# tspooner/rl_markets

Measured on NVIDIA H100. Metric: env steps/sec (batched LOBs), higher is better.
Workload: dtype f64

## Files before the change

rl_markets_b200/csrc/rlm_api.cu:

```cuda
#include <cuda_runtime.h>
#include <math.h>
#include <stdio.h>
#include <string.h>
#include <algorithm>
#include <mutex>
#include <string>
#include <vector>

#include "rlm.h"
#include "rlm_flow_tables.h"
#include "rlm_rndseq.h"
#include "rlm_kernels.h"
#include <limits.h>
#include <stddef.h>
#include <stdlib.h>

static thread_local std::string g_err;
static int fail(int code, const std::string& msg) { g_err = msg; return code; }
int rlm_set_error_(int code, const std::string& msg) { return fail(code, msg); }
#define CK(expr)                                                                                      \
  do {                                                                                                \
    cudaError_t _e = (expr);                                                                          \
    if (_e != cudaSuccess) return fail((_e == cudaErrorNoDevice || _e == cudaErrorInsufficientDriver) ? RLM_ERR_NO_DEVICE : RLM_ERR_CUDA, \
                                       std::string(#expr) + ": " + cudaGetErrorString(_e));          \
// ... 33 lines not shown
  long long launches = 0;
  double alpha = 0, eps = 0, tau = 1.0;
  int n_sub = 1;
  struct TickGraph { int chunk; DynParams d; cudaGraphExec_t exec; };
  std::vector<TickGraph> graphs;
  bool use_graphs = true, graph_warm = false;
  bool staged = false;
  cudaStream_t sub_stream[RLM_MAX_SUB] = {};
  cudaEvent_t ev_fork = nullptr, ev_join[RLM_MAX_SUB] = {};
  bool rounds = false;
  bool in_rounds = false;
  bool rounds_auto = false;
  int run_seq = 0;
  int round_streams = 1;
  int* h_live = nullptr;
  cudaEvent_t ev_live[RLM_MAX_SUB][2] = {};
  long long rounds_launched = 0, rounds_calls = 0;
};

static const rlm_handle_s* g_params_owner = nullptr;
static std::recursive_mutex g_api_mu;
#define API_LOCK std::lock_guard<std::recursive_mutex> api_lock_(g_api_mu)

static int split_scratch(rlm_handle_s* h, size_t bytes) {
  if (bytes > h->gather_cap) {
    CK(cudaStreamSynchronize(h->stream));
    cudaFree(h->d_gather); if (h->h_gather) cudaFreeHost(h->h_gather);
    h->d_gather = nullptr; h->h_gather = nullptr; h->gather_cap = 0;
    CK(cudaMalloc(&h->d_gather, bytes));
    CK(cudaMallocHost(&h->h_gather, bytes));
// ... 253 lines not shown
  int rc = upload_params(h);
  if (rc != RLM_OK) return rc;
  CK(rlm_launch_init(h->ptr, cfg->n_envs, 0, h->stream));
  CK(rlm_launch_seed(h->ptr, cfg->n_envs, cfg->random_seed, h->stream));
  if (cfg->random_init) CK(rlm_launch_random_init(h->ptr, h->n_policies, h->stream));
  h->alpha = cfg->alpha_start;
  h->eps = (double)cfg->eps_init;
  h->tau = (double)cfg->tau_init;
  memset(&h->dyn, 0, sizeof(h->dyn));
#ifdef RLM_TIMING
  if (const char* s = getenv("RLM_DEBUG_FLAGS")) h->dyn.debug_flags = atoi(s);
#endif
  if (const char* s = getenv("RLM_ENV_HASH")) h->dyn.env_hash = atoi(s) != 0;
  if (const char* s = getenv("RLM_ROUND_CAP")) h->dyn.round_cap = std::max(0, atoi(s));
  CK(cudaDeviceGetAttribute(&h->n_sms, cudaDevAttrMultiProcessorCount, cfg->device));
  CK(cudaMalloc(&h->ptr.ready, (size_t)cfg->n_envs * 4));
  CK(cudaMalloc(&h->ptr.hsum, (size_t)cfg->n_envs * 3 * 32 * 8));
  h->ready_cap = RLM_READY_CAP;
  CK(cudaMalloc(&h->ptr.ready_count, (size_t)2 * RLM_LIVE_OFF * 4));
  CK(cudaMemset(h->ptr.ready_count, 0, (size_t)2 * RLM_LIVE_OFF * 4));
  CK(cudaMalloc(&h->ptr.runctl, sizeof(RunCtl)));
  CK(cudaMemset(h->ptr.runctl, 0, sizeof(RunCtl)));
  CK(cudaMallocHost(&h->h_live, RLM_MAX_SUB * 2 * sizeof(int)));
  for (int s = 0; s < RLM_MAX_SUB; ++s)
    for (int i = 0; i < 2; ++i) CK(cudaEventCreateWithFlags(&h->ev_live[s][i], cudaEventDisableTiming));
  if (const char* s = getenv("RLM_ROUND_STREAMS")) { const int v = atoi(s); if (v >= 1 && v <= RLM_MAX_SUB) h->round_streams = v; }
  h->n_sub = 1;
  h->staged = !h->hp.is_double && !cfg->shared_policy && cfg->memory_size * 8 <= 65536 && (cfg->memory_size % 2) == 0;
  if (const char* s = getenv("RLM_STAGED")) h->staged = h->staged && atoi(s) != 0;
  if (cfg->n_envs > 16384 && !h->staged) h->agent_variant = 3;
  if (const char* s = getenv("RLM_AGENT_VARIANT")) { const int v = atoi(s); h->agent_variant = (v == 1 || v == 3) ? v : 4; }
  if (cfg->memory_size > (1LL << 27) && h->agent_variant == 4) h->agent_variant = 3;
  if (const char* s = getenv("RLM_GRAPHS")) h->use_graphs = atoi(s) != 0;
  if (const char* s = getenv("RLM_SUBBATCHES")) { const int v = atoi(s); if (v >= 1 && v <= RLM_MAX_SUB) h->n_sub = cfg->shared_policy ? 1 : v; }
  if (std::max(h->n_sub, h->round_streams) > 1) {
// ... 21 lines not shown
    const int resident = rlm_run_max_resident_ctas(p.scratch_bytes, h->n_sms);
    const int n_env_ctas = (cfg->n_envs + 127) / 128;
    int want = (cfg->n_envs + 3) / 4;
    int cap = resident - std::min(n_env_ctas, std::max(resident / 4, 1));
    h->n_agent_ctas = std::max(1, std::min(want, cap));
    if (const char* s = getenv("RLM_AGENT_CTAS")) { int v = atoi(s); if (v > 0 && v < resident) h->n_agent_ctas = v; }
    if (const char* s = getenv("RLM_ENGINE")) h->engine = (s[0] == 'p') ? 0 : ((s[0] == 'f') ? 2 : ((s[0] == 'F') ? 3 : 1));
    h->env_variant = (cfg->n_envs > 16384) ? 1 : 0;
    if (const char* s = getenv("RLM_ENV_VARIANT")) h->env_variant = atoi(s) ? 1 : 0;
    h->rounds = false;
    h->rounds_auto = !cfg->shared_policy && h->env_variant == 0 && h->engine == 1 && !getenv("RLM_ENGINE") && cfg->algorithm < RLM_ALGO_R_LEARN;
    if (const char* s = getenv("RLM_ROUNDS")) {
      h->rounds = atoi(s) != 0 && !cfg->shared_policy && h->env_variant == 0;
      h->rounds_auto = false;
    }
    if (!getenv("RLM_ROUND_CAP")) h->dyn.round_cap = 3;
    if (const char* s = getenv("RLM_PDL")) rlm_set_pdl(atoi(s));
    if (const char* s = getenv("RLM_AGENT_VARIANT")) { const int v = atoi(s); h->agent_variant = (v == 1 || v == 3) ? v : 4; }
    if (cfg->memory_size > (1LL << 27)) {
      if (h->agent_variant == 4) h->agent_variant = 3;
      if (h->engine == 3) h->engine = 1;
    }
  }
  if (cfg->source == RLM_SOURCE_TAPE) {
    if (h->engine != 1) return fail(RLM_ERR_UNSUPPORTED, "the tape source runs on the tick-synchronous and round-paced engines (RLM_ENGINE=F|f|p read the stream source only)");
    h->dyn.tape_l2 = 1;
    if (const char* s = getenv("RLM_TAPE_PREFETCH")) h->dyn.tape_l2 = atoi(s) != 0;
  }
  cudaDeviceSetLimit(cudaLimitMaxL2FetchGranularity, 32);
  CK(cudaStreamSynchronize(h->stream));
  return RLM_OK;
}
// ... 2 lines not shown
  API_LOCK;
  if (!h) return RLM_OK;
  cudaSetDevice(h->cfg.device);
  cudaStreamSynchronize(h->stream);
  cudaFree(h->ptr.env); cudaFree(h->ptr.theta); cudaFree(h->ptr.theta_b); cudaFree(h->ptr.dtheta);
  cudaFree(h->ptr.trace_f); cudaFree(h->ptr.trace_e); cudaFree(h->ptr.mt_pol); cudaFree(h->ptr.mt_agt);
  cudaFree(h->ptr.records); cudaFree(h->ptr.record_count); cudaFree(h->ptr.counters);
  cudaFree(h->d_gather); if (h->h_gather) cudaFreeHost(h->h_gather);
  if (h->copy_stream) { cudaStreamSynchronize(h->copy_stream); cudaStreamDestroy(h->copy_stream); }
  for (int i = 0; i < 2; ++i) {
    cudaFree(h->d_stream[i]);
    if (h->ev_copied[i]) cudaEventDestroy(h->ev_copied[i]);
    if (h->ev_consumed[i]) cudaEventDestroy(h->ev_consumed[i]);
  }
  cudaFree(h->ptr.ready); cudaFree(h->ptr.ready_count); cudaFree(h->ptr.occ); cudaFree(h->ptr.hsum);
  cudaFree(h->ptr.runctl); if (h->h_live) cudaFreeHost(h->h_live);
  cudaFree((void*)h->ptr.tape); cudaFree(h->ptr.tape_cur); cudaFree(h->ptr.tape_lo);
  for (auto& es : h->ev_live) for (auto e : es) if (e) cudaEventDestroy(e);
  cudaFree(h->ptr.q_slots); cudaFree(h->ptr.ag_done); cudaFree(h->d_qctl);
  for (auto e : h->ev) cudaEventDestroy(e);
  for (auto& g : h->graphs) cudaGraphExecDestroy(g.exec);
  if (h->ev_fork) cudaEventDestroy(h->ev_fork);
  for (int s = 0; s < RLM_MAX_SUB; ++s) {
    if (h->sub_stream[s]) { cudaStreamSynchronize(h->sub_stream[s]); cudaStreamDestroy(h->sub_stream[s]); }
    if (h->ev_join[s]) cudaEventDestroy(h->ev_join[s]);
  }
  if (h->own_stream && h->stream) cudaStreamDestroy(h->stream);
  if (g_params_owner == h) g_params_owner = nullptr;
  delete h;
  return RLM_OK;
}
// ... 201 lines not shown
  CK(rlm_launch_runctl(h->ptr, rc, h->stream));
  const int S = h->profile ? 1 : std::max(1, std::min(h->round_streams, (B + 255) / 256));
  int sub0[RLM_MAX_SUB + 1];
  {
    const int per = (((B + S - 1) / S) + 31) & ~31;
    for (int s = 0; s <= S; ++s) sub0[s] = std::min(B, s * per);
  }
  int G = n_ticks >= 512 ? 32 : (n_ticks >= 128 ? 16 : 8);
  G = std::min(std::min(G, n_ticks + 1), h->ready_cap);
  const bool graphs = h->use_graphs && h->graph_warm && !h->profile;
  h->graph_warm = true;
  if (h->profile) while ((int)h->ev.size() < 3 * G) { cudaEvent_t e; CK(cudaEventCreate(&e)); h->ev.push_back(e); }
  DynParams dts[RLM_MAX_SUB];
  DevPtrs pss[RLM_MAX_SUB];
  cudaGraphExec_t exec[RLM_MAX_SUB] = {};
  if (S > 1) CK(cudaEventRecord(h->ev_fork, h->stream));
  for (int s = 0; s < S; ++s) {
    cudaStream_t st = S > 1 ? h->sub_stream[s] : h->stream;
    if (S > 1) CK(cudaStreamWaitEvent(st, h->ev_fork, 0));
    DynParams& dt = dts[s];
    dt = d;
    dt.n_ticks = 0; dt.stream_off = 0; dt.stream_ticks = 0; dt.env0 = sub0[s]; dt.n_sub = sub0[s + 1] - sub0[s]; dt.sub_idx = s;
    DevPtrs& ps = pss[s];
    ps = h->ptr;
    ps.stream = nullptr;
    ps.ready = h->ptr.ready + sub0[s];
    ps.ready_count = h->ptr.ready_count + (size_t)s * h->ready_cap;
    if (!graphs || dt.n_sub <= 0) continue;
    for (auto& g : h->graphs)
      if (g.chunk == -G && memcmp(&g.d, &dt, sizeof(DynParams)) == 0) exec[s] = g.exec;
    if (!exec[s]) {
      if (h->graphs.size() >= 24) {
        CK(cudaStreamSynchronize(h->stream));
        for (auto& g : h->graphs) cudaGraphExecDestroy(g.exec);
        h->graphs.clear();
        for (int q = 0; q < s; ++q) exec[q] = nullptr;
      }
      cudaGraph_t graph = nullptr;
      CK(cudaStreamBeginCapture(st, cudaStreamCaptureModeThreadLocal));
      cudaError_t ce = cudaMemsetAsync(ps.ready_count, 0, (size_t)G * 4, st);
      if (ce == cudaSuccess) ce = cudaMemsetAsync(ps.ready_count + RLM_LIVE_OFF, 0, (size_t)G * 4, st);
      for (int r = 0; r < G && ce == cudaSuccess; ++r) {
        ce = rlm_launch_env_round(ps, dt, dt.n_sub, r, st);
        if (ce == cudaSuccess) ce = launch_agent_on(h, ps, dt, r, 0, st);
      }
      cudaError_t ce2 = cudaStreamEndCapture(st, &graph);
      if (ce != cudaSuccess || ce2 != cudaSuccess) { if (graph) cudaGraphDestroy(graph); CK(ce != cudaSuccess ? ce : ce2); }
      ce = cudaGraphInstantiate(&exec[s], graph, 0);
      cudaGraphDestroy(graph);
      CK(ce);
      h->graphs.push_back({-G, dt, exec[s]});
    }
  }
  const int max_groups = (n_ticks + 1 + G - 1) / G + 1;
  bool live[RLM_MAX_SUB];
  int n_live = 0;
  for (int s = 0; s < S; ++s) { live[s] = sub0[s + 1] > sub0[s]; n_live += live[s] ? 1 : 0; }
  h->rounds_calls++;
  for (int k = 0; k <= max_groups && n_live > 0; ++k) {
    for (int s = 0; s < S && k < max_groups; ++s) {
      if (!live[s]) continue;
      cudaStream_t st = S > 1 ? h->sub_stream[s] : h->stream;
      if (exec[s]) CK(cudaGraphLaunch(exec[s], st));
      else {
        CK(cudaMemsetAsync(pss[s].ready_count, 0, (size_t)G * 4, st));
        CK(cudaMemsetAsync(pss[s].ready_count + RLM_LIVE_OFF, 0, (size_t)G * 4, st));
        for (int r = 0; r < G; ++r) {
          if (h->profile) CK(cudaEventRecord(h->ev[3 * r], st));
          CK(rlm_launch_env_round(pss[s], dts[s], dts[s].n_sub, r, st));
          if (h->profile) CK(cudaEventRecord(h->ev[3 * r + 1], st));
          CK(launch_agent_on(h, pss[s], dts[s], r, 0, st));
          if (h->profile) CK(cudaEventRecord(h->ev[3 * r + 2], st));
        }
        if (h->profile) {
          std::vector<int> cnt(2 * G);
          CK(cudaStreamSynchronize(st));
          CK(cudaMemcpy(cnt.data(), pss[s].ready_count, (size_t)G * 4, cudaMemcpyDeviceToHost));
          CK(cudaMemcpy(cnt.data() + G, pss[s].ready_count + RLM_LIVE_OFF, (size_t)G * 4, cudaMemcpyDeviceToHost));
          for (int r = 0; r < G; ++r) {
            float a = 0, b = 0;
            CK(cudaEventElapsedTime(&a, h->ev[3 * r], h->ev[3 * r + 1]));
            CK(cudaEventElapsedTime(&b, h->ev[3 * r + 1], h->ev[3 * r + 2]));
            if (cnt[G + r] > 0) { h->prof_env_ms += a; h->prof_env_launches++; }
            if (cnt[r] > 0) { h->prof_agent_ms += b; h->prof_agent_launches++; }
          }
        }
// ... 654 lines not shown
```

rl_markets_b200/csrc/rlm_kernels.cu:

```cuda
#include <cuda_runtime.h>
#include <stdint.h>
#define RLM_TABLE_QUAL static __device__ const
#include "rlm_flow_tables.h"
#include "rlm_rndseq.h"
#include "rlm_agent.cuh"
#include <cstdio>
#include "rlm_kernels.h"
#define RLM_ENVT_CARVEOUT_DEFAULT 30
#define RLM_SMEM_CARVEOUT 88

#define SCR_Q 0
#define SCR_SS (SCR_Q + 8 * 2 * RLM_MAX_ACTIONS)
#define SCR_IDX (SCR_SS + 4 * SS_SLOTS)
#define SCR_VBUF (SCR_IDX + 4 * 3 * RLM_MAX_ACTIONS * 32)
#define AG_BYTES ((sizeof(AgentD) + 15) & ~(size_t)15)
size_t rlm_scratch_bytes(int is_double) {
  return ((size_t)SCR_VBUF + (size_t)(is_double ? 2 : 1) * RLM_MAX_ACTIONS * VROW * 8 + 15) & ~(size_t)15;
}
size_t rlm_agent_smem_bytes(int warps_per_cta, int scratch_bytes) {
  return (size_t)warps_per_cta * (AG_BYTES + (size_t)scratch_bytes);
}

#define PDL_PROLOGUE() do { asm volatile("griddepcontrol.launch_dependents;" ::: "memory"); asm volatile("griddepcontrol.wait;" ::: "memory"); } while (0)
static bool g_use_pdl = false;
void rlm_set_pdl(int on) { g_use_pdl = on != 0; }
template <typename... KArgs, typename... Args>
static cudaError_t launch_pdl(void (*kernel)(KArgs...), int grid, int block, size_t smem, cudaStream_t st, Args... args) {
  cudaLaunchConfig_t cfg = {};
  cfg.gridDim = dim3(grid); cfg.blockDim = dim3(block); cfg.dynamicSmemBytes = smem; cfg.stream = st;
  cudaLaunchAttribute at[1];
  at[0].id = cudaLaunchAttributeProgrammaticStreamSerialization;
  at[0].val.programmaticStreamSerializationAllowed = g_use_pdl ? 1 : 0;
  cfg.attrs = at; cfg.numAttrs = 1;
  return cudaLaunchKernelEx(&cfg, kernel, args...);
}

#ifdef RLM_TIMING
__device__ unsigned long long g_klog[256][8][2][2];
__device__ __forceinline__ unsigned long long gtime() { unsigned long long t; asm volatile("mov.u64 %0, %%globaltimer;" : "=l"(t)); return t; }
#define KLOG_BEGIN(kind) do { if (threadIdx.x == 0 && tslot < 256) atomicMin(&g_klog[tslot][D.sub_idx & 7][kind][0], gtime()); } while (0)
#define KLOG_END(kind) do { if (threadIdx.x == 0 && tslot < 256) atomicMax(&g_klog[tslot][D.sub_idx & 7][kind][1], gtime()); } while (0)
extern "C" int rlm_debug_klog(unsigned long long* out, int reset) {
  cudaDeviceSynchronize();
  if (out && cudaMemcpyFromSymbol(out, g_klog, sizeof(g_klog)) != cudaSuccess) return -1;
  if (reset) {
    static unsigned long long init[256][8][2][2];
    for (auto& a : init) for (auto& b : a) for (auto& c : b) { c[0] = ~0ull; c[1] = 0ull; }
// ... 730 lines not shown
            }
          }
        }
        if (lane == 0) e.ag.hs_valid = 1;
      }
    } else if (ready == 1 && D.backtest) {
      if (lane < P.n_state_vars) e.ag.to_vars[lane] = (float)get_variable(e, ring, P.state_vars[lane]);
    }
  }
  __syncwarp();
  return ready;
}

template <bool TAPE>
__global__ void __launch_bounds__(ENVW_WARPS * 32) rlm_env_kernel_w(DevPtrs ptr, DynParams D, int tslot, int only_begin) {
  PDL_PROLOGUE();
  extern __shared__ __align__(16) unsigned char smem[];
  const int tid = threadIdx.x, lane = tid & 31, warp = tid >> 5;
  const int env = D.env0 + blockIdx.x * (blockDim.x >> 5) + warp;
  if (!only_begin) KLOG_BEGIN(0);
  if (env >= (D.n_sub > 0 ? D.env0 + D.n_sub : P.n_envs)) return;
  const EnvWarp w = envw_carve(smem + (size_t)warp * envw_warp_bytes());
  EnvHdr& e = *w.e;
  EnvHdr* g = (EnvHdr*)(ptr.env + (size_t)env * P.env_stride);
  double* ring = (double*)((unsigned char*)g + sizeof(EnvHdr));
  if (only_begin && !g->ag.need_begin) return;
  const bool tape = TAPE && !only_begin;
  int2 tc = make_int2(0, 0);
  unsigned tape_word = 0;
  if (tape) tape_word = envw_stage_in_tape(&e, g, ptr, env, lane, D.tape_l2 != 0, tc);
  else envw_stage_in(&e, g, lane);
// ... 22 lines not shown
  }
  __syncwarp();
  envw_stage_out(g, &e, lane);
  if (!only_begin) KLOG_END(0);
  if (lane == 0) {
    if (ready >= 0) ptr.ready[atomicAdd(&ptr.ready_count[tslot], 1)] = env;
    if (D.hold && ready < 0 && e.phase != PH_DONE && !starved) atomicAdd(&ptr.counters[5], 1ull);
    if (ticked) atomicAdd(&ptr.counters[0], 1ull);
    const unsigned errs = (unsigned)(e.err | e.ag.err);
    if (errs) atomicOr(&ptr.counters[4], (unsigned long long)errs);
  }
}

template <bool TAPE>
__global__ void __launch_bounds__(ENVW_WARPS * 32, 4) rlm_env_round_kernel(DevPtrs ptr, DynParams D, int tslot) {
  PDL_PROLOGUE();
  extern __shared__ __align__(16) unsigned char smem[];
  const int tid = threadIdx.x, lane = tid & 31, warp = tid >> 5;
  const int env = D.env0 + blockIdx.x * (blockDim.x >> 5) + warp;
  KLOG_BEGIN(0);
  if (env >= (D.n_sub > 0 ? D.env0 + D.n_sub : P.n_envs)) return;
  int* live_count = ptr.ready_count + RLM_LIVE_OFF;
  if (tslot > 0 && __ldcg(live_count + tslot - 1) == 0) return;
  const int4 rc4 = __ldg((const int4*)ptr.runctl);
  const RunCtl rc = {rc4.x, rc4.y, rc4.z, rc4.w, nullptr, 0};
  DevPtrs pt = ptr;
  pt.stream = (const rlm_tick_msg*)__ldg((const unsigned long long*)ptr.runctl + 2);
  const EnvWarp w = envw_carve(smem + (size_t)warp * envw_warp_bytes());
  EnvHdr& e = *w.e;
  EnvHdr* g = (EnvHdr*)(ptr.env + (size_t)env * P.env_stride);
  double* ring = (double*)((unsigned char*)g + sizeof(EnvHdr));
  const bool tape = TAPE;
  int2 tc = make_int2(0, 0);
  unsigned tape_word = 0;
  if (tape) tape_word = envw_stage_in_tape(&e, g, ptr, env, lane, false, tc);
  else envw_stage_in(&e, g, lane);
  __syncwarp();
  if (e.phase == PH_DONE) return;
// ... 19 lines not shown
    }
    ++pos; ++n_run;
    if (ready >= 0) break;
  }
  if (lane == 0) {
    e.run_id = rc.run_id; e.run_pos = pos;
    if (tape) {
      ptr.tape_cur[env].x = tc.x;
      if (D.tape_l2 && tc.x < tc.y) asm volatile("prefetch.global.L2 [%0];" ::"l"(ptr.tape + tc.x));
    }
  }
  __syncwarp();
  envw_stage_out(g, &e, lane);
  KLOG_END(0);
  if (lane == 0) {
    if (ready >= 0) ptr.ready[atomicAdd(&ptr.ready_count[tslot], 1)] = env;
    if (ready >= 0 || (e.phase != PH_DONE && pos < rc.n_ticks && !starved)) atomicAdd(&live_count[tslot], 1);
    if (ticked) atomicAdd(&ptr.counters[0], (unsigned long long)ticked);
    const unsigned errs = (unsigned)(e.err | e.ag.err);
    if (errs) atomicOr(&ptr.counters[4], (unsigned long long)errs);
  }
}
__global__ void rlm_runctl_kernel(RunCtl* dst, RunCtl v) { *dst = v; }

__device__ __forceinline__ void emit_record(const DevPtrs& ptr, const EnvHdr* g, int env, const AgentD& ag, const double* theta_a,
                                         const float* vars, int lane) {
  const int* tf = ptr.trace_f + (size_t)env * P.trace_cap;
  const float* te = ptr.trace_e + (size_t)env * P.trace_cap;
  unsigned long long h = trace_hash(tf, te, theta_a, ag.n_traces, lane);
  if (lane == 0) {
    int c = ptr.record_count[env];
    if (c < P.record_cap) {
// ... 420 lines not shown
  int f[RLM_MAX_ACTIONS];
  const unsigned long long base = a3_hash(rlm_rndseq_table, ag.to_vars, P.n_state_vars, false, warp, lane, f);
  if (P.occ_smem_words) { asm volatile("cp.async.wait_all;" ::: "memory"); __syncthreads(); }
  a3_gather(theta_a, theta_b, occ, occ_sm, f, warp, lane, V);
  __syncthreads();
  if (warp == 0) {
    double qa = 0.0, qb = 0.0;
    if (lane < P.n_actions) a3_sums(V, theta_b != nullptr, lane, qa, qb);
    backtest_advance(ptr, g, env, ag, theta_a, kind, qa, qb, base, lane, steps_done);
  }
  return (int)steps_done;
}

template <bool EXTRAS>
__global__ void __launch_bounds__(A3_WARPS * 32, 10) rlm_agent3_kernel(DevPtrs ptr, DynParams D, int tslot, int stage) {
  PDL_PROLOGUE();
  extern __shared__ __align__(16) unsigned char smem[];
  const int tid = threadIdx.x, lane = tid & 31, warp = tid >> 5;
  AgentD& ag = *(AgentD*)smem;
  unsigned char* sb = smem + AG_BYTES;
  double* q_pre_a = (double*)(sb + A3_Q);
  double* q_pre_b = q_pre_a + RLM_MAX_ACTIONS;
  int* sset = (int*)(sb + A3_SS);
  double* dec = (double*)(sb + A3_DEC);
  double* V = (double*)(sb + A3_V);
  unsigned* occ_s = (unsigned*)(sb + a3_occ_offset(P.is_double));
  const unsigned* rnd = rlm_rndseq_table;
  const int A = P.n_actions;
  const int n_ready = ptr.ready_count[tslot];
  unsigned long long steps_done = 0, sum_z = 0;
#pragma unroll 1
// ... 145 lines not shown
}

cudaError_t rlm_launch_agent3(const DevPtrs& ptr, const DynParams& D, int n_envs, int is_double, int occ_smem_words, int tslot, int n_sms,
                              int stage, int full, cudaStream_t st) {
  const size_t smem = rlm_agent3_smem_bytes(is_double, occ_smem_words);
  static size_t attr_smem[2] = {0, 0};
  if (smem > attr_smem[full ? 1 : 0]) {
    cudaError_t e = full ? cudaFuncSetAttribute(rlm_agent3_kernel<true>, cudaFuncAttributeMaxDynamicSharedMemorySize, (int)smem)
                         : cudaFuncSetAttribute(rlm_agent3_kernel<false>, cudaFuncAttributeMaxDynamicSharedMemorySize, (int)smem);
    if (e != cudaSuccess) return e;
    attr_smem[full ? 1 : 0] = smem;
  }
  int grid = n_envs;
  const int cap = n_sms * 16;
  if (grid > cap) grid = cap;
  if (full) return launch_pdl(rlm_agent3_kernel<true>, grid, A3_WARPS * 32, smem, st, ptr, D, tslot, stage);
  return launch_pdl(rlm_agent3_kernel<false>, grid, A3_WARPS * 32, smem, st, ptr, D, tslot, stage);
}

template <int WARPS>
__global__ void __launch_bounds__(WARPS * 32) rlm_agent_kernel(DevPtrs ptr, DynParams D, int tslot, int stage) {
  extern __shared__ __align__(16) unsigned char smem[];
  const int tid = threadIdx.x, lane = tid & 31, warp = tid >> 5;
  unsigned char* wbase = smem + (size_t)warp * (AG_BYTES + P.scratch_bytes);
  AgentD& ag = *(AgentD*)wbase;
  unsigned char* scratch = wbase + AG_BYTES;
  const int n_ready = ptr.ready_count[tslot];
  unsigned long long steps_done = 0, sum_z = 0;
#pragma unroll 1
  for (int idx = blockIdx.x * WARPS + warp; idx < n_ready; idx += gridDim.x * WARPS)
    agent_process_env(ptr, D, ptr.ready[idx], ag, std_scratch(scratch), lane, steps_done, sum_z, stage, nullptr);
  if (lane == 0 && (steps_done | sum_z)) {
// ... 334 lines not shown
    else rlm_env_kernel<T, false><<<(n_envs + T - 1) / T, T, 0, st>>>(ptr, D, tslot, only_begin);
    return cudaGetLastError();
  }
  const int W = envw_warps_per_cta();
  const size_t smem = (size_t)W * envw_warp_bytes();
  auto kern = tape ? rlm_env_kernel_w<true> : rlm_env_kernel_w<false>;
  static bool attr[2] = {false, false};
  if (!attr[tape]) {
    if (smem > 48 * 1024) {
      cudaError_t e = cudaFuncSetAttribute(kern, cudaFuncAttributeMaxDynamicSharedMemorySize, (int)smem);
      if (e != cudaSuccess) return e;
    }
    cudaFuncSetAttribute(kern, cudaFuncAttributePreferredSharedMemoryCarveout, envw_carveout());
    attr[tape] = true;
  }
  return launch_pdl(kern, (n_envs + W - 1) / W, W * 32, smem, st, ptr, D, tslot, only_begin);
}

cudaError_t rlm_launch_env_round(const DevPtrs& ptr, const DynParams& D, int n_envs, int tslot, cudaStream_t st) {
  const int W = envw_warps_per_cta();
  const size_t smem = (size_t)W * envw_warp_bytes();
  const bool tape = ptr.tape_cur != nullptr;
  auto kern = tape ? rlm_env_round_kernel<true> : rlm_env_round_kernel<false>;
  static bool attr[2] = {false, false};
  if (!attr[tape]) {
    if (smem > 48 * 1024) {
      cudaError_t e = cudaFuncSetAttribute(kern, cudaFuncAttributeMaxDynamicSharedMemorySize, (int)smem);
      if (e != cudaSuccess) return e;
    }
    cudaFuncSetAttribute(kern, cudaFuncAttributePreferredSharedMemoryCarveout, envw_carveout());
    attr[tape] = true;
  }
  return launch_pdl(kern, (n_envs + W - 1) / W, W * 32, smem, st, ptr, D, tslot);
}
cudaError_t rlm_launch_runctl(const DevPtrs& ptr, const RunCtl& v, cudaStream_t st) {
  rlm_runctl_kernel<<<1, 1, 0, st>>>(ptr.runctl, v);
  return cudaGetLastError();
}

cudaError_t rlm_launch_agent(const DevPtrs& ptr, const DynParams& D, int n_envs, int scratch_bytes, int tslot, int n_sms, int stage, cudaStream_t st) {
  const int W = 8;
  size_t smem = rlm_agent_smem_bytes(W, scratch_bytes);
  static size_t attr_smem = 0;
  if (smem > attr_smem) {
    cudaError_t e = cudaFuncSetAttribute(rlm_agent_kernel<W>, cudaFuncAttributeMaxDynamicSharedMemorySize, (int)smem);
    if (e != cudaSuccess) return e;
    attr_smem = smem;
  }
// ... 112 lines not shown
```

rl_markets_b200/csrc/rlm_kernels.h:

```cpp
#pragma once
#include <cuda_runtime.h>
#include "rlm_types.h"

size_t rlm_scratch_bytes(int is_double);
size_t rlm_agent_smem_bytes(int warps_per_cta, int scratch_bytes);
cudaError_t rlm_upload_params(const DevParams* p);
cudaError_t rlm_launch_env(const DevPtrs& ptr, const DynParams& D, int n_envs, int tslot, int only_begin, int variant, cudaStream_t st);
cudaError_t rlm_launch_env_round(const DevPtrs& ptr, const DynParams& D, int n_envs, int tslot, cudaStream_t st);
cudaError_t rlm_launch_runctl(const DevPtrs& ptr, const RunCtl& v, cudaStream_t st);
cudaError_t rlm_launch_agent(const DevPtrs& ptr, const DynParams& D, int n_envs, int scratch_bytes, int tslot, int n_sms, int stage, cudaStream_t st);
cudaError_t rlm_launch_agent3(const DevPtrs& ptr, const DynParams& D, int n_envs, int is_double, int occ_smem_words, int tslot, int n_sms, int stage, int full,
                              cudaStream_t st);
cudaError_t rlm_launch_learn(const DevPtrs& ptr, const DynParams& D, int n_envs, int is_double, int tslot, int n_sms, int stage, int expected_steps, cudaStream_t st);
cudaError_t rlm_launch_learn_staged(const DevPtrs& ptr, const DynParams& D, int n_envs, long long memory_size, int tslot, int n_sms, cudaStream_t st);
cudaError_t rlm_launch_fused2(const DevPtrs& ptr, const DynParams& D, int n_envs, int is_double, cudaStream_t st);
cudaError_t rlm_launch_apply_dtheta(double* theta, double* dtheta, long long n, int n_sms, cudaStream_t st);
size_t rlm_fused_smem_bytes(int is_double);
cudaError_t rlm_launch_fused(const DevPtrs& ptr, const DynParams& D, int n_envs, int is_double, cudaStream_t st);
cudaError_t rlm_launch_run(const DevPtrs& ptr, const DynParams& D, int n_envs, int scratch_bytes, int n_agent_ctas, cudaStream_t st);
int rlm_run_max_resident_ctas(int scratch_bytes, int n_sms);
cudaError_t rlm_launch_act(const DevPtrs& ptr, const DynParams& D, int n_envs, int* actions, cudaStream_t st);
cudaError_t rlm_launch_apply(const DevPtrs& ptr, const DynParams& D, int n_envs, const int* actions, cudaStream_t st);
cudaError_t rlm_launch_step_out(const DevPtrs& ptr, int n_envs, double* reward, unsigned char* terminal, double* delta, cudaStream_t st);
cudaError_t rlm_launch_count_nonzero(const double* theta, long long M, int n_policies, int* out, cudaStream_t st);
cudaError_t rlm_launch_init(const DevPtrs& ptr, int n_envs, int mode, cudaStream_t st);
cudaError_t rlm_launch_seed(const DevPtrs& ptr, int n_envs, unsigned seed, cudaStream_t st);
cudaError_t rlm_launch_random_init(const DevPtrs& ptr, int n_policies, cudaStream_t st);
void rlm_set_pdl(int on);
cudaError_t rlm_launch_gather(const DevPtrs& ptr, int n_envs, int what, void* out, cudaStream_t st);
cudaError_t rlm_launch_clear_traces(const DevPtrs& ptr, int n_envs, cudaStream_t st);
cudaError_t rlm_launch_test_to_ticks(const double* px, int n, int* out);
cudaError_t rlm_launch_test_to_price(const int* t, int n, double* out);
cudaError_t rlm_launch_test_tiles(const float* vars, int n, int* out);
cudaError_t rlm_launch_test_learner_tiles(int form, const float* vars, int n, int* out);
cudaError_t rlm_launch_test_order(long long size, long long q_head, const rlm_order_op* ops, int n_ops, rlm_order_state* out);
cudaError_t rlm_launch_test_rolling_mean(const double* vals, int n, double* out, double* ring_mem, EnvHdr* e);
```

rl_markets_b200/csrc/rlm_learn.cuh:

```cuda
#pragma once

#ifndef LN_WARPS
#define LN_WARPS 3
#endif
#define LN_MIN_CTAS (15 / LN_WARPS)
#ifdef RLM_TIMING
#define LPH(i) do { if (lane == 0 && tp_idx < 4096) g_phase_clk[tp_idx * 16 + (i)] = clock64(); } while (0)
#else
#define LPH(i) do { } while (0)
#endif
#define LN_VROW 98
#define LN_AG_BYTES 704

__host__ __device__ inline size_t ln_v_bytes(int is_double) { return (size_t)(is_double ? 2 : 1) * RLM_MAX_ACTIONS * LN_VROW * 8; }
#ifndef UT_LOG2
#define UT_LOG2 10
#endif
#define UT_SLOTS (1 << UT_LOG2)
#define UT_MAX_ENTRIES (UT_SLOTS / 2)
__host__ __device__ inline size_t ln_scratch_bytes(int is_double) {
  return (ln_v_bytes(is_double) + TT_SLOTS * 4 + 2 * UT_SLOTS * 4 + 8 * 2 * RLM_MAX_ACTIONS + 48 + 15) & ~(size_t)15;
}
__host__ __device__ inline size_t ln_warp_bytes(int is_double) { return (size_t)LN_AG_BYTES + ln_scratch_bytes(is_double); }
static_assert(sizeof(AgentD) <= LN_AG_BYTES, "agent block outgrew its shared-memory slot");
// ... 425 lines not shown
    __stcg(dst + lane, src[lane]);
    if (lane + 32 < N16) __stcg(dst + lane + 32, src[lane + 32]);
    if (lane < 3 && ag.need_begin) {
      int k = ag.mt_pol_idx; if (k >= 312) k -= 312;
      int kk = k + (lane == 0 ? 0 : (lane == 1 ? 1 : 156)); if (kk >= 312) kk -= 312;
      asm volatile("prefetch.global.L2 [%0];" ::"l"(ptr.mt_pol + (size_t)env * 312 + kk));
    }
  }
  __syncwarp();
  LPH(12);
#ifdef RLM_TIMING
  if (lane == 0 && tp_idx < 4096) { unsigned s_; asm volatile("mov.u32 %0, %%smid;" : "=r"(s_)); g_phase_sm[tp_idx] = s_; }
#endif
}

template <bool DBL>
__global__ void __launch_bounds__(LN_WARPS * 32, LN_MIN_CTAS) rlm_learn_kernel(DevPtrs ptr, DynParams D, int tslot, int stage) {
  extern __shared__ __align__(16) unsigned char smem[];
  const int lane = threadIdx.x & 31, warp = threadIdx.x >> 5;
  unsigned char* wsm = smem + (size_t)warp * ln_warp_bytes(DBL ? 1 : 0);
  for (int i = threadIdx.x; i < 64; i += LN_WARPS * 32) asm volatile("prefetch.global.L1 [%0];" ::"l"(rlm_rndseq_table + i * 32));
  const int n_ready = ptr.ready_count[tslot];
  unsigned long long steps_done = 0, sum_z = 0;
  if (n_ready > (int)blockIdx.x) KLOG_BEGIN(1);
  const int C = gridDim.x;
#pragma unroll 1
  for (int idx = warp * C + blockIdx.x; idx < n_ready; idx += LN_WARPS * C)
    ln_step<DBL, false, 27>(ptr, D, ptr.ready[idx], *(AgentD*)wsm, wsm + LN_AG_BYTES, nullptr, lane, stage, steps_done, sum_z, idx);
  if (steps_done) KLOG_END(1);
  if (lane == 0 && (steps_done | sum_z)) {
    atomicAdd(&ptr.counters[1], steps_done);
    atomicAdd(&ptr.counters[2], sum_z);
  }
}

cudaError_t rlm_launch_learn(const DevPtrs& ptr, const DynParams& D, int n_envs, int is_double, int tslot, int n_sms, int stage, int expected_steps, cudaStream_t st) {
  const size_t smem = LN_WARPS * ln_warp_bytes(is_double);
  static size_t attr_smem[2] = {0, 0};
  if (smem > attr_smem[is_double ? 1 : 0]) {
    cudaError_t e = is_double ? cudaFuncSetAttribute(rlm_learn_kernel<true>, cudaFuncAttributeMaxDynamicSharedMemorySize, (int)smem)
                              : cudaFuncSetAttribute(rlm_learn_kernel<false>, cudaFuncAttributeMaxDynamicSharedMemorySize, (int)smem);
    if (e != cudaSuccess) return e;
    if (is_double) cudaFuncSetAttribute(rlm_learn_kernel<true>, cudaFuncAttributePreferredSharedMemoryCarveout, RLM_SMEM_CARVEOUT);
// ... 150 lines not shown
#pragma unroll
    for (int j = 0; j < 8; ++j) nxt[j] = w * tab[ii[j]];
#pragma unroll
    for (int j = 0; j < 8; ++j) acc += cur[j];
#pragma unroll
    for (int j = 0; j < 8; ++j) cur[j] = nxt[j];
  }
  return acc;
}
__device__ __noinline__ double ls_sums(const double* tab, const unsigned short* idx, int lane) {
  ASSUME_SHARED(tab); ASSUME_SHARED(idx);
  return (lane < P.n_actions) ? ls_chain(tab, idx + lane * LS_IROW) : 0.0;
}

__global__ void __launch_bounds__(32, 6) rlm_learn_staged_kernel(DevPtrs ptr, DynParams D, int tslot) {
  extern __shared__ __align__(16) unsigned char smem[];
  const int lane = threadIdx.x;
  unsigned long long* mbar = (unsigned long long*)smem;
  AgentD& ag = *(AgentD*)(smem + 16);
  unsigned short* idx_s = (unsigned short*)(smem + 16 + LN_AG_BYTES);
  int* tt = (int*)(idx_s + RLM_MAX_ACTIONS * LS_IROW);
  double* q_pre_a = (double*)(tt + TT_SLOTS);
  double* q_pre_b = q_pre_a + RLM_MAX_ACTIONS;
  double* dec = q_pre_b + RLM_MAX_ACTIONS;
  double* tab = (double*)(smem + ((ls_fixed_bytes() + 15) & ~(size_t)15));
  const unsigned mbar_a = smem_u32(mbar), tab_a = smem_u32(tab);
  const unsigned table_bytes = (unsigned)(P.memory_size * 8);
  if (lane == 0) {
    asm volatile("mbarrier.init.shared::cta.b64 [%0], 1;" ::"r"(mbar_a) : "memory");
    asm volatile("fence.mbarrier_init.release.cluster;" ::: "memory");
// ... 155 lines not shown
      q = ls_sums(tab, idx_s, lane);
      if (lane < A) { ag.q_from[lane] = q; ag.qb_from[lane] = 0.0; }
    }
    __syncwarp();
    {
      int4* dst = (int4*)&g->ag;
      const int4* src = (const int4*)&ag;
      __stcg(dst + lane, src[lane]);
      if (lane + 32 < N16) __stcg(dst + lane + 32, src[lane + 32]);
      if (lane < 3 && ag.need_begin) {
        int k = ag.mt_pol_idx; if (k >= 312) k -= 312;
        int kk = k + (lane == 0 ? 0 : (lane == 1 ? 1 : 156)); if (kk >= 312) kk -= 312;
        asm volatile("prefetch.global.L2 [%0];" ::"l"(ptr.mt_pol + (size_t)env * 312 + kk));
      }
    }
  }
  if (lane == 0 && (steps_done | sum_z)) {
    atomicAdd(&ptr.counters[1], steps_done);
    atomicAdd(&ptr.counters[2], sum_z);
  }
}

__host__ inline bool rlm_learn_staged_ok(long long memory_size, int is_double, int shared_policy) {
  return !is_double && !shared_policy && memory_size * 8 <= 65536 && memory_size <= 65536 && (memory_size % 2) == 0;
}
cudaError_t rlm_launch_learn_staged(const DevPtrs& ptr, const DynParams& D, int n_envs, long long memory_size, int tslot, int n_sms, cudaStream_t st) {
  const size_t smem = ls_smem_bytes(memory_size);
  static size_t attr_smem = 0;
  static int per_sm = 1;
  if (smem > attr_smem) {
// ... 14 lines not shown
```

rl_markets_b200/csrc/rlm_types.h:

```cpp
#pragma once
#include <stdint.h>
#include "rlm.h"

#define RLM_NWIN 10
enum { W_MID = 0, W_VLT, W_VNUM, W_VDEN, W_SPREAD, W_TP, W_ASKTX, W_BIDTX, W_PNLUP, W_PNLDN };

enum { PH_PREOPEN = 0, PH_WARMUP = 1, PH_RUN = 2, PH_DONE = 3 };

enum {
  ERR_BAD_PRICE = 1,
  ERR_TICK_RANGE = 2,
  ERR_TRACE_OVERFLOW = 4,
  ERR_INVALID_STATE = 8,
  ERR_STREAM_UNDERRUN = 16
};

struct OrderD {
  double price;
  long long size, q_head, q_tail, executed, initial_queue;
  int live;
  int transactions;
};

struct SideD {
// ... 106 lines not shown
  int env0;
  int backtest;
  int n_sub;
  int sub_idx;
  int debug_flags;
  int env_hash;
  int round_cap;
  int ctl_stream;
  int hold;
  int tape_l2;
};

#define RLM_MAX_SUB 8
#define RLM_READY_CAP 256
#define RLM_LIVE_OFF (RLM_MAX_SUB * RLM_READY_CAP)

struct RunCtl { int run_id, n_ticks, stream_off, stream_ticks; const rlm_tick_msg* stream; long long pad; };

struct DevPtrs {
  unsigned char* env;
  double* theta;
  double* theta_b;
  double* dtheta;
  int* trace_f;
  float* trace_e;
  unsigned long long* mt_pol;
  unsigned long long* mt_agt;
  const rlm_tick_msg* stream;
  rlm_step_record* records;
  int* record_count;
  unsigned long long* counters;
  unsigned* occ;
  unsigned long long* hsum;
  int* ready;
  int* ready_count;
  int* q_slots;
  unsigned* q_head;
  unsigned* q_tail;
  unsigned* env_warps_done;
  int* q_done;
  int* ag_done;
  int q_size;
  int pad;
  RunCtl* runctl;
  const rlm_tick_msg* tape;
  int2* tape_cur;
  int* tape_lo;
};
```

Baseline: 12.29 million.

## Overlap env rounds with learn kernel via per-env handoff flags and PDL

Adds per-env learn request/done counters so that the next env round kernel can launch early under programmatic dependent launch and spin-wait only on the envs whose learn step is still pending. The env round kernel now compacts its grid to the ready and waiting envs of the previous round, using double-buffered ready lists, instead of scanning all envs. It also removes the global PDL toggle, raises the default round cap from 3 to 4, and adds memsets and allocations for the new wait counters. Spin-waiting with nanosleep risks contention or deadlock if the learn kernel cannot become co-resident, and it adds fence and atomic overhead.

```diff
diff --git a/rl_markets_b200/csrc/rlm_api.cu b/rl_markets_b200/csrc/rlm_api.cu
--- a/rl_markets_b200/csrc/rlm_api.cu
+++ b/rl_markets_b200/csrc/rlm_api.cu
@@ -71,6 +71,7 @@
   int run_seq = 0;
   int round_streams = 1;
   int* h_live = nullptr;
+  unsigned* learn_req = nullptr;
   cudaEvent_t ev_live[RLM_MAX_SUB][2] = {};
   long long rounds_launched = 0, rounds_calls = 0;
 };
@@ -354,11 +355,13 @@
   if (const char* s = getenv("RLM_ENV_HASH")) h->dyn.env_hash = atoi(s) != 0;
   if (const char* s = getenv("RLM_ROUND_CAP")) h->dyn.round_cap = std::max(0, atoi(s));
   CK(cudaDeviceGetAttribute(&h->n_sms, cudaDevAttrMultiProcessorCount, cfg->device));
-  CK(cudaMalloc(&h->ptr.ready, (size_t)cfg->n_envs * 4));
+  CK(cudaMalloc(&h->ptr.ready, (size_t)2 * cfg->n_envs * 4));
   CK(cudaMalloc(&h->ptr.hsum, (size_t)cfg->n_envs * 3 * 32 * 8));
   h->ready_cap = RLM_READY_CAP;
-  CK(cudaMalloc(&h->ptr.ready_count, (size_t)2 * RLM_LIVE_OFF * 4));
-  CK(cudaMemset(h->ptr.ready_count, 0, (size_t)2 * RLM_LIVE_OFF * 4));
+  CK(cudaMalloc(&h->ptr.ready_count, (size_t)3 * RLM_LIVE_OFF * 4));
+  CK(cudaMemset(h->ptr.ready_count, 0, (size_t)3 * RLM_LIVE_OFF * 4));
+  CK(cudaMalloc(&h->learn_req, (size_t)2 * cfg->n_envs * sizeof(unsigned)));
+  CK(cudaMemset(h->learn_req, 0, (size_t)2 * cfg->n_envs * sizeof(unsigned)));
   CK(cudaMalloc(&h->ptr.runctl, sizeof(RunCtl)));
   CK(cudaMemset(h->ptr.runctl, 0, sizeof(RunCtl)));
   CK(cudaMallocHost(&h->h_live, RLM_MAX_SUB * 2 * sizeof(int)));
@@ -410,8 +413,7 @@
       h->rounds = atoi(s) != 0 && !cfg->shared_policy && h->env_variant == 0;
       h->rounds_auto = false;
     }
-    if (!getenv("RLM_ROUND_CAP")) h->dyn.round_cap = 3;
-    if (const char* s = getenv("RLM_PDL")) rlm_set_pdl(atoi(s));
+    if (!getenv("RLM_ROUND_CAP")) h->dyn.round_cap = 4;
     if (const char* s = getenv("RLM_AGENT_VARIANT")) { const int v = atoi(s); h->agent_variant = (v == 1 || v == 3) ? v : 4; }
     if (cfg->memory_size > (1LL << 27)) {
       if (h->agent_variant == 4) h->agent_variant = 3;
@@ -444,7 +446,7 @@
     if (h->ev_consumed[i]) cudaEventDestroy(h->ev_consumed[i]);
   }
   cudaFree(h->ptr.ready); cudaFree(h->ptr.ready_count); cudaFree(h->ptr.occ); cudaFree(h->ptr.hsum);
-  cudaFree(h->ptr.runctl); if (h->h_live) cudaFreeHost(h->h_live);
+  cudaFree(h->ptr.runctl); if (h->h_live) cudaFreeHost(h->h_live); cudaFree(h->learn_req);
   cudaFree((void*)h->ptr.tape); cudaFree(h->ptr.tape_cur); cudaFree(h->ptr.tape_lo);
   for (auto& es : h->ev_live) for (auto e : es) if (e) cudaEventDestroy(e);
   cudaFree(h->ptr.q_slots); cudaFree(h->ptr.ag_done); cudaFree(h->d_qctl);
@@ -676,6 +678,13 @@
   DynParams dts[RLM_MAX_SUB];
   DevPtrs pss[RLM_MAX_SUB];
   cudaGraphExec_t exec[RLM_MAX_SUB] = {};
+  const bool handoff = !h->profile && h->agent_variant == 4 && !d.backtest && h->cfg.algorithm < RLM_ALGO_R_LEARN;
+  auto round_ptrs = [&](int s, int r) {
+    DevPtrs pr = pss[s];
+    pr.ready = h->ptr.ready + (size_t)(r & 1) * B + sub0[s];
+    pr.ready_prev = h->ptr.ready + (size_t)((r + 1) & 1) * B + sub0[s];
+    return pr;
+  };
   if (S > 1) CK(cudaEventRecord(h->ev_fork, h->stream));
   for (int s = 0; s < S; ++s) {
     cudaStream_t st = S > 1 ? h->sub_stream[s] : h->stream;
@@ -686,8 +695,9 @@
     DevPtrs& ps = pss[s];
     ps = h->ptr;
     ps.stream = nullptr;
-    ps.ready = h->ptr.ready + sub0[s];
     ps.ready_count = h->ptr.ready_count + (size_t)s * h->ready_cap;
+    ps.learn_req = handoff ? h->learn_req : nullptr;
+    ps.learn_done = handoff ? h->learn_req + B : nullptr;
     if (!graphs || dt.n_sub <= 0) continue;
     for (auto& g : h->graphs)
       if (g.chunk == -G && memcmp(&g.d, &dt, sizeof(DynParams)) == 0) exec[s] = g.exec;
@@ -702,9 +712,11 @@
       CK(cudaStreamBeginCapture(st, cudaStreamCaptureModeThreadLocal));
       cudaError_t ce = cudaMemsetAsync(ps.ready_count, 0, (size_t)G * 4, st);
       if (ce == cudaSuccess) ce = cudaMemsetAsync(ps.ready_count + RLM_LIVE_OFF, 0, (size_t)G * 4, st);
+      if (ce == cudaSuccess) ce = cudaMemsetAsync(ps.ready_count + RLM_WAIT_OFF, 0, (size_t)G * 4, st);
       for (int r = 0; r < G && ce == cudaSuccess; ++r) {
-        ce = rlm_launch_env_round(ps, dt, dt.n_sub, r, st);
-        if (ce == cudaSuccess) ce = launch_agent_on(h, ps, dt, r, 0, st);
+        const DevPtrs pr = round_ptrs(s, r);
+        ce = rlm_launch_env_round(pr, dt, dt.n_sub, r, st);
+        if (ce == cudaSuccess) ce = launch_agent_on(h, pr, dt, r, 0, st);
       }
       cudaError_t ce2 = cudaStreamEndCapture(st, &graph);
       if (ce != cudaSuccess || ce2 != cudaSuccess) { if (graph) cudaGraphDestroy(graph); CK(ce != cudaSuccess ? ce : ce2); }
@@ -727,11 +739,13 @@
       else {
         CK(cudaMemsetAsync(pss[s].ready_count, 0, (size_t)G * 4, st));
         CK(cudaMemsetAsync(pss[s].ready_count + RLM_LIVE_OFF, 0, (size_t)G * 4, st));
+        CK(cudaMemsetAsync(pss[s].ready_count + RLM_WAIT_OFF, 0, (size_t)G * 4, st));
         for (int r = 0; r < G; ++r) {
+          const DevPtrs pr = round_ptrs(s, r);
           if (h->profile) CK(cudaEventRecord(h->ev[3 * r], st));
-          CK(rlm_launch_env_round(pss[s], dts[s], dts[s].n_sub, r, st));
+          CK(rlm_launch_env_round(pr, dts[s], dts[s].n_sub, r, st));
           if (h->profile) CK(cudaEventRecord(h->ev[3 * r + 1], st));
-          CK(launch_agent_on(h, pss[s], dts[s], r, 0, st));
+          CK(launch_agent_on(h, pr, dts[s], r, 0, st));
           if (h->profile) CK(cudaEventRecord(h->ev[3 * r + 2], st));
         }
         if (h->profile) {
diff --git a/rl_markets_b200/csrc/rlm_kernels.cu b/rl_markets_b200/csrc/rlm_kernels.cu
--- a/rl_markets_b200/csrc/rlm_kernels.cu
+++ b/rl_markets_b200/csrc/rlm_kernels.cu
@@ -21,16 +21,13 @@
   return (size_t)warps_per_cta * (AG_BYTES + (size_t)scratch_bytes);
 }
 
-#define PDL_PROLOGUE() do { asm volatile("griddepcontrol.launch_dependents;" ::: "memory"); asm volatile("griddepcontrol.wait;" ::: "memory"); } while (0)
-static bool g_use_pdl = false;
-void rlm_set_pdl(int on) { g_use_pdl = on != 0; }
 template <typename... KArgs, typename... Args>
-static cudaError_t launch_pdl(void (*kernel)(KArgs...), int grid, int block, size_t smem, cudaStream_t st, Args... args) {
+static cudaError_t launch_pdl(bool pdl, void (*kernel)(KArgs...), int grid, int block, size_t smem, cudaStream_t st, Args... args) {
   cudaLaunchConfig_t cfg = {};
   cfg.gridDim = dim3(grid); cfg.blockDim = dim3(block); cfg.dynamicSmemBytes = smem; cfg.stream = st;
   cudaLaunchAttribute at[1];
   at[0].id = cudaLaunchAttributeProgrammaticStreamSerialization;
-  at[0].val.programmaticStreamSerializationAllowed = g_use_pdl ? 1 : 0;
+  at[0].val.programmaticStreamSerializationAllowed = pdl ? 1 : 0;
   cfg.attrs = at; cfg.numAttrs = 1;
   return cudaLaunchKernelEx(&cfg, kernel, args...);
 }
@@ -791,7 +788,6 @@
 
 template <bool TAPE>
 __global__ void __launch_bounds__(ENVW_WARPS * 32) rlm_env_kernel_w(DevPtrs ptr, DynParams D, int tslot, int only_begin) {
-  PDL_PROLOGUE();
   extern __shared__ __align__(16) unsigned char smem[];
   const int tid = threadIdx.x, lane = tid & 31, warp = tid >> 5;
   const int env = D.env0 + blockIdx.x * (blockDim.x >> 5) + warp;
@@ -844,14 +840,31 @@
 
 template <bool TAPE>
 __global__ void __launch_bounds__(ENVW_WARPS * 32, 4) rlm_env_round_kernel(DevPtrs ptr, DynParams D, int tslot) {
-  PDL_PROLOGUE();
   extern __shared__ __align__(16) unsigned char smem[];
   const int tid = threadIdx.x, lane = tid & 31, warp = tid >> 5;
-  const int env = D.env0 + blockIdx.x * (blockDim.x >> 5) + warp;
+  const int i = blockIdx.x * (blockDim.x >> 5) + warp;
+  const int n_sub = D.n_sub > 0 ? D.n_sub : P.n_envs;
   KLOG_BEGIN(0);
-  if (env >= (D.n_sub > 0 ? D.env0 + D.n_sub : P.n_envs)) return;
-  int* live_count = ptr.ready_count + RLM_LIVE_OFF;
-  if (tslot > 0 && __ldcg(live_count + tslot - 1) == 0) return;
+  int env;
+  if (tslot == 0) {
+    if (i >= n_sub) return;
+    env = D.env0 + i;
+  } else {
+    const int n_wait = __ldcg(ptr.ready_count + RLM_WAIT_OFF + tslot - 1);
+    if (i < n_wait) env = __ldcg(ptr.ready_prev + n_sub - 1 - i);
+    else if (i - n_wait < __ldcg(ptr.ready_count + tslot - 1)) env = __ldcg(ptr.ready_prev + i - n_wait);
+    else return;
+  }
+  if (ptr.learn_done) {
+    const unsigned req = __ldcg(ptr.learn_req + env);
+    unsigned done, ns = 64;
+    asm volatile("ld.acquire.gpu.global.u32 %0, [%1];" : "=r"(done) : "l"(ptr.learn_done + env) : "memory");
+    while (done != req) {
+      __nanosleep(ns);
+      if (ns < 1024) ns *= 2;
+      asm volatile("ld.acquire.gpu.global.u32 %0, [%1];" : "=r"(done) : "l"(ptr.learn_done + env) : "memory");
+    }
+  }
   const int4 rc4 = __ldg((const int4*)ptr.runctl);
   const RunCtl rc = {rc4.x, rc4.y, rc4.z, rc4.w, nullptr, 0};
   DevPtrs pt = ptr;
@@ -901,8 +914,14 @@
   envw_stage_out(g, &e, lane);
   KLOG_END(0);
   if (lane == 0) {
-    if (ready >= 0) ptr.ready[atomicAdd(&ptr.ready_count[tslot], 1)] = env;
-    if (ready >= 0 || (e.phase != PH_DONE && pos < rc.n_ticks && !starved)) atomicAdd(&live_count[tslot], 1);
+    if (ready >= 0) {
+      if (ptr.learn_req) ptr.learn_req[env] += 1;
+      ptr.ready[atomicAdd(&ptr.ready_count[tslot], 1)] = env;
+    }
+    if (ready >= 0 || (e.phase != PH_DONE && pos < rc.n_ticks && !starved)) {
+      atomicAdd(&ptr.ready_count[RLM_LIVE_OFF + tslot], 1);
+      if (ready < 0) ptr.ready[(D.n_sub > 0 ? D.n_sub : P.n_envs) - 1 - atomicAdd(&ptr.ready_count[RLM_WAIT_OFF + tslot], 1)] = env;
+    }
     if (ticked) atomicAdd(&ptr.counters[0], (unsigned long long)ticked);
     const unsigned errs = (unsigned)(e.err | e.ag.err);
     if (errs) atomicOr(&ptr.counters[4], (unsigned long long)errs);
@@ -1353,7 +1372,6 @@
 
 template <bool EXTRAS>
 __global__ void __launch_bounds__(A3_WARPS * 32, 10) rlm_agent3_kernel(DevPtrs ptr, DynParams D, int tslot, int stage) {
-  PDL_PROLOGUE();
   extern __shared__ __align__(16) unsigned char smem[];
   const int tid = threadIdx.x, lane = tid & 31, warp = tid >> 5;
   AgentD& ag = *(AgentD*)smem;
@@ -1529,8 +1547,9 @@
   int grid = n_envs;
   const int cap = n_sms * 16;
   if (grid > cap) grid = cap;
-  if (full) return launch_pdl(rlm_agent3_kernel<true>, grid, A3_WARPS * 32, smem, st, ptr, D, tslot, stage);
-  return launch_pdl(rlm_agent3_kernel<false>, grid, A3_WARPS * 32, smem, st, ptr, D, tslot, stage);
+  if (full) rlm_agent3_kernel<true><<<grid, A3_WARPS * 32, smem, st>>>(ptr, D, tslot, stage);
+  else rlm_agent3_kernel<false><<<grid, A3_WARPS * 32, smem, st>>>(ptr, D, tslot, stage);
+  return cudaGetLastError();
 }
 
 template <int WARPS>
@@ -1895,7 +1914,8 @@
     cudaFuncSetAttribute(kern, cudaFuncAttributePreferredSharedMemoryCarveout, envw_carveout());
     attr[tape] = true;
   }
-  return launch_pdl(kern, (n_envs + W - 1) / W, W * 32, smem, st, ptr, D, tslot, only_begin);
+  kern<<<(n_envs + W - 1) / W, W * 32, smem, st>>>(ptr, D, tslot, only_begin);
+  return cudaGetLastError();
 }
 
 cudaError_t rlm_launch_env_round(const DevPtrs& ptr, const DynParams& D, int n_envs, int tslot, cudaStream_t st) {
@@ -1912,7 +1932,7 @@
     cudaFuncSetAttribute(kern, cudaFuncAttributePreferredSharedMemoryCarveout, envw_carveout());
     attr[tape] = true;
   }
-  return launch_pdl(kern, (n_envs + W - 1) / W, W * 32, smem, st, ptr, D, tslot);
+  return launch_pdl(ptr.learn_done != nullptr && tslot > 0, kern, (n_envs + W - 1) / W, W * 32, smem, st, ptr, D, tslot);
 }
 cudaError_t rlm_launch_runctl(const DevPtrs& ptr, const RunCtl& v, cudaStream_t st) {
   rlm_runctl_kernel<<<1, 1, 0, st>>>(ptr.runctl, v);
diff --git a/rl_markets_b200/csrc/rlm_kernels.h b/rl_markets_b200/csrc/rlm_kernels.h
--- a/rl_markets_b200/csrc/rlm_kernels.h
+++ b/rl_markets_b200/csrc/rlm_kernels.h
@@ -26,7 +26,6 @@
 cudaError_t rlm_launch_init(const DevPtrs& ptr, int n_envs, int mode, cudaStream_t st);
 cudaError_t rlm_launch_seed(const DevPtrs& ptr, int n_envs, unsigned seed, cudaStream_t st);
 cudaError_t rlm_launch_random_init(const DevPtrs& ptr, int n_policies, cudaStream_t st);
-void rlm_set_pdl(int on);
 cudaError_t rlm_launch_gather(const DevPtrs& ptr, int n_envs, int what, void* out, cudaStream_t st);
 cudaError_t rlm_launch_clear_traces(const DevPtrs& ptr, int n_envs, cudaStream_t st);
 cudaError_t rlm_launch_test_to_ticks(const double* px, int n, int* out);
diff --git a/rl_markets_b200/csrc/rlm_learn.cuh b/rl_markets_b200/csrc/rlm_learn.cuh
--- a/rl_markets_b200/csrc/rlm_learn.cuh
+++ b/rl_markets_b200/csrc/rlm_learn.cuh
@@ -463,8 +463,21 @@
 #endif
 }
 
+__device__ __forceinline__ void ln_handoff_open(const DevPtrs& ptr) {
+  if (!ptr.learn_done) return;
+  asm volatile("griddepcontrol.wait;" ::: "memory");
+  asm volatile("griddepcontrol.launch_dependents;" ::: "memory");
+}
+__device__ __forceinline__ void ln_handoff_publish(const DevPtrs& ptr, int env, int lane) {
+  if (!ptr.learn_done) return;
+  __threadfence();
+  __syncwarp();
+  if (lane == 0) asm volatile("st.release.gpu.global.u32 [%0], %1;" ::"l"(ptr.learn_done + env), "r"(__ldcg(ptr.learn_req + env)) : "memory");
+}
+
 template <bool DBL>
 __global__ void __launch_bounds__(LN_WARPS * 32, LN_MIN_CTAS) rlm_learn_kernel(DevPtrs ptr, DynParams D, int tslot, int stage) {
+  ln_handoff_open(ptr);
   extern __shared__ __align__(16) unsigned char smem[];
   const int lane = threadIdx.x & 31, warp = threadIdx.x >> 5;
   unsigned char* wsm = smem + (size_t)warp * ln_warp_bytes(DBL ? 1 : 0);
@@ -474,8 +487,11 @@
   if (n_ready > (int)blockIdx.x) KLOG_BEGIN(1);
   const int C = gridDim.x;
 #pragma unroll 1
-  for (int idx = warp * C + blockIdx.x; idx < n_ready; idx += LN_WARPS * C)
-    ln_step<DBL, false, 27>(ptr, D, ptr.ready[idx], *(AgentD*)wsm, wsm + LN_AG_BYTES, nullptr, lane, stage, steps_done, sum_z, idx);
+  for (int idx = warp * C + blockIdx.x; idx < n_ready; idx += LN_WARPS * C) {
+    const int env = ptr.ready[idx];
+    ln_step<DBL, false, 27>(ptr, D, env, *(AgentD*)wsm, wsm + LN_AG_BYTES, nullptr, lane, stage, steps_done, sum_z, idx);
+    ln_handoff_publish(ptr, env, lane);
+  }
   if (steps_done) KLOG_END(1);
   if (lane == 0 && (steps_done | sum_z)) {
     atomicAdd(&ptr.counters[1], steps_done);
@@ -656,6 +672,7 @@
 }
 
 __global__ void __launch_bounds__(32, 6) rlm_learn_staged_kernel(DevPtrs ptr, DynParams D, int tslot) {
+  ln_handoff_open(ptr);
   extern __shared__ __align__(16) unsigned char smem[];
   const int lane = threadIdx.x;
   unsigned long long* mbar = (unsigned long long*)smem;
@@ -841,6 +858,7 @@
         asm volatile("prefetch.global.L2 [%0];" ::"l"(ptr.mt_pol + (size_t)env * 312 + kk));
       }
     }
+    ln_handoff_publish(ptr, env, lane);
   }
   if (lane == 0 && (steps_done | sum_z)) {
     atomicAdd(&ptr.counters[1], steps_done);
diff --git a/rl_markets_b200/csrc/rlm_types.h b/rl_markets_b200/csrc/rlm_types.h
--- a/rl_markets_b200/csrc/rlm_types.h
+++ b/rl_markets_b200/csrc/rlm_types.h
@@ -144,6 +144,7 @@
 #define RLM_MAX_SUB 8
 #define RLM_READY_CAP 256
 #define RLM_LIVE_OFF (RLM_MAX_SUB * RLM_READY_CAP)
+#define RLM_WAIT_OFF (2 * RLM_LIVE_OFF)
 
 struct RunCtl { int run_id, n_ticks, stream_off, stream_ticks; const rlm_tick_msg* stream; long long pad; };
 
@@ -164,6 +165,9 @@
   unsigned long long* hsum;
   int* ready;
   int* ready_count;
+  const int* ready_prev;
+  unsigned* learn_req;
+  unsigned* learn_done;
   int* q_slots;
   unsigned* q_head;
   unsigned* q_tail;
```

Result: faster. 12.91 million, median of 6 (+5.1%).
